# rland93/rrtplanner

Measured on NVIDIA B200. Metric: RRT* plans/sec (512x512 grid, n=5000), higher is better.
Workload: dtype f64

## Files before the change

profiles/region_profile.py:

```python
import csv, re, subprocess, sys, tempfile, os
sass_csv, so, cubin_name, func_pat = sys.argv[1:5]
tmp = tempfile.mkdtemp()
subprocess.check_call(["cuobjdump", "-xelf", "all", os.path.abspath(so)], cwd=tmp, stdout=subprocess.DEVNULL)
dis = subprocess.run(["nvdisasm", "-g", "-c", os.path.join(tmp, cubin_name)], capture_output=True, text=True).stdout
line_of = {}; cur=None; infunc=False
for ln in dis.splitlines():
    m = re.match(r"\s*\.section\s+\.text\.(\S+?),", ln)
    if m: infunc = func_pat in m.group(1); continue
    if not infunc: continue
    m = re.search(r'//## File "([^"]+)", line (\d+)(?: inlined at "([^"]+)", line (\d+))?', ln)
    if m:
        f, l = os.path.basename(m.group(1)), int(m.group(2))
        if m.group(3): of, ol = os.path.basename(m.group(3)), int(m.group(4))
        else: of, ol = None, None
        cur = (f, l, of, ol); continue
    m = re.match(r"\s*/\*([0-9a-f]{4,})\*/\s+(.*?);", ln)
    if m: line_of[int(m.group(1), 16)] = cur
rows = list(csv.reader(open(sass_csv))); hdr = rows[1]
ci, cs = hdr.index("Instructions Executed"), hdr.index("# Samples")
base = int(rows[2][0], 16)
regions = [("setup+prologue", 0, 178), ("owner:pickup", 179, 191), ("owner:scan", 192, 239), ("owner:nearest/dup/walk", 240, 287), ("owner:costing+cands", 288, 378), ("owner:record", 379, 392), ("commit", 393, 528), ("round end", 529, 543), ("goal+out", 544, 700)]
agg = {r[0]: [0, 0] for r in regions}; agg["other"] = [0, 0]; tot=[0,0]
unk = {}
for r in rows[2:]:
    try: off = int(r[0], 16) - base; n, s = int(r[ci]), int(r[cs])
    except Exception: continue
    k = line_of.get(off)
    line = None
    if k:
        if k[0] == "plan_grid.cuh": line = k[1]
        elif k[2] == "plan_grid.cuh": line = k[3]
    name = "other"
    if line is not None:
        for nm, a, b in regions:
            if a <= line <= b: name = nm
    else:
        unk[k] = unk.get(k, 0) + n
    agg[name][0] += n; agg[name][1] += s; tot[0]+=n; tot[1]+=s
for nm, (n, s) in agg.items(): print(f"{nm:28s} instr {n/1e6:8.1f}M {100*n/tot[0]:5.1f}%   samples {s:7d} {100*s/tot[1]:5.1f}%")
for k, n in sorted(unk.items(), key=lambda kv: -kv[1])[:12]: print("   other:", k, f"{n/1e6:.1f}M")
```

rrtplanner_b200/csrc/plan.cu:

```cuda
#include <cstdlib>

#include "plan_common.cuh"

namespace rrtk {

int scan_launch_standard(const PlanParams &, int, int, int, int, size_t, cudaStream_t);
int scan_launch_star(const PlanParams &, int, int, int, int, size_t, cudaStream_t);
int scan_launch_informed(const PlanParams &, int, int, int, int, size_t, cudaStream_t);
int scan_occupancy_standard(int, int, int, size_t);
int scan_occupancy_star(int, int, int, size_t);
int scan_occupancy_informed(int, int, int, size_t);
int grid_launch(int, int, const PlanParams &, int, size_t, cudaStream_t);
int grid_occupancy(int, int, bool, size_t);
int wide_plan_launch(int, const uint32_t *, int, int, const rrtk_plan_desc *, int, int, double, double, const int16_t *,
                     const double *, int16_t *, double *, int32_t *, int64_t *, double *, int, int, int, cudaStream_t);
int wide_plan_footprint(int, int, int, int, int, int, int, int *, int *);

struct ScanShape {
    int T, K, hit_words, tail_bytes, sbits, steps_max, list_cap, blocks_per_sm, two_per_sm;
    size_t smem;
};

static int env_int(const char *name, int dflt)
{
    const char *s = getenv(name);
    return (s && *s) ? atoi(s) : dflt;
}

#ifndef RRTK_MINB128
#define RRTK_MINB128 7
#endif
static int scan_min_blocks(int T) { return T <= 64 ? 12 : T <= 128 ? RRTK_MINB128 : T <= 160 ? 5 : T <= 256 ? 3 : 1; }

struct GridShape {
    int xb, yb, bshift, bshy, nbx, nby, rad, list_cap, blocks_per_sm, K, kb, ent_words, off_list, off_bstart;
    uint32_t near_ok2;
    size_t smem;
};

static int bits_for(int v) { int b = 0; while ((1 << b) <= v) ++b; return b; }

static bool grid_shape(int kind, int W, int H, int n, double r_rewire, int threads, int optin, int sm_smem, GridShape *out)
{
    const char *impl = getenv("RRTK_PLAN_IMPL");
    if (impl && (impl[0] == 'w' || impl[0] == 's')) return false;
#ifdef RRTK_GRID_OPT_IN
    if (!(impl && impl[0] == 'g')) return false;
#endif
    if (kind != RRTK_STANDARD && kind != RRTK_STAR) return false;
    if (threads != 0 && threads != 128) return false;
    if (env_int("RRTK_PLAN_T", 0) != 0) return false;
    if (n < 256 && !(impl && impl[0] == 'g')) return false;
    GridShape g;
    g.K = env_int("RRTK_GRID_K", 16);
    if (g.K != 8 && g.K != 16) return false;
    g.xb = bits_for(W - 1); g.yb = bits_for(H - 1);
    const int ib = 32 - g.xb - g.yb;
    if (ib < 1 || ib > 31 || (long long)n >= (1ll << ib) - 1) return false;
    g.bshift = env_int("RRTK_GRID_BSX", 5); g.bshy = env_int("RRTK_GRID_BSY", 2);
    for (;;) {
        g.nbx = (W + (1 << g.bshift) - 1) >> g.bshift; g.nby = (H + (1 << g.bshy) - 1) >> g.bshy;
        if (g.nbx * g.nby <= 2048 && g.nbx * g.nby + 1 <= n) break;
        if (g.bshift >= 15) return false;
        if (g.bshy < g.bshift) ++g.bshy; else ++g.bshift;
    }
    const double r = kind == RRTK_STAR ? (r_rewire > 0.0 ? r_rewire : 0.0) : 0.0;
    double rad = ceil(r);
    if (rad < (double)(1 << g.bshift)) rad = (double)(1 << g.bshift);
    if (rad > 32768.0) rad = 32768.0;
    g.rad = (int)rad;
    g.near_ok2 = (uint32_t)(rad * rad);
    int cap = env_int("RRTK_PLAN_CAP", 256);
    const int need = (n + 1 + 31) & ~31;
    g.list_cap = kind == RRTK_STANDARD ? 0 : (cap < need ? cap : need);
    g.ent_words = (n + 1 + 31) & ~31;
    g.off_list = 4 * g.ent_words;
    g.off_bstart = g.off_list + 4 * 4 * g.list_cap;
    g.smem = (size_t)g.off_bstart + (((size_t)2 * (g.nbx * g.nby + 1) + 15) & ~(size_t)15);
    g.kb = bits_for(n);
    {
        const long long d2max = (long long)(W - 1) * (W - 1) + (long long)(H - 1) * (H - 1);
        if (g.kb >= 32 || d2max >= (1ll << (32 - g.kb)) - 1 || env_int("RRTK_GRID_KEY32", 1) == 0) g.kb = 0;
    }
    if (g.smem > (size_t)optin - 4096) return false;
    int b = grid_occupancy(kind, g.K, g.kb > 0, g.smem);
    if (b <= 0) {
        b = (int)((size_t)sm_smem / (g.smem + 3072));
        if (b > 7) b = 7;
    }
    g.blocks_per_sm = b < 1 ? 1 : b;
    *out = g;
    return true;
}

static bool scan_shape(int kind, int W, int H, int n, int threads, int optin, int sm_smem, ScanShape *out)
{
    const char *impl = getenv("RRTK_PLAN_IMPL");
    if (impl && impl[0] == 'w') return false;
    if (n + 1 > 65535) return false;
    ScanShape s;
    s.K = env_int("RRTK_PLAN_K", 8);
    if (s.K != 4 && s.K != 8 && s.K != 16) return false;
    int T = threads > 0 ? threads : env_int("RRTK_PLAN_T", 0);
    if (T <= 0) T = n < 2048 ? 64 : n < 5120 ? 128 : n < 32768 ? 256 : 512;
    if (T != 64 && T != 128 && T != 160 && T != 256 && T != 512) return false;
    const int rows = (n + 1 + T - 1) / T;
    s.T = T;
    s.hit_words = (rows + 31) / 32;
    if (s.hit_words > 4) return false;
    s.sbits = s.hit_words == 1 ? 5 : s.hit_words == 2 ? 6 : 7;
    const long long side = W > H ? W : H;
    if (((2 * side * side) << s.sbits) > (1ll << 29)) return false;
    s.steps_max = (rows + 3) / 4;
    int cap = env_int("RRTK_PLAN_CAP", kind == RRTK_INFORMED ? 448 : 256);
    const int need = (n + 1 + 31) & ~31;
    s.list_cap = kind == RRTK_STANDARD ? 0 : (cap < need ? cap : need);
    s.smem = (size_t)4 * 4 * T * s.steps_max;
    const int tail_rows = rows - 32 * (s.hit_words - 1);
    s.tail_bytes = tail_rows <= 8 ? 1 : tail_rows <= 16 ? 2 : 4;
    if (kind != RRTK_STANDARD)
        s.smem += (size_t)4 * (s.hit_words - 1) * s.K * T + (((size_t)s.tail_bytes * s.K * T + 3) & ~(size_t)3) + (size_t)2 * (T / 32) * s.list_cap;
    s.smem = (s.smem + 15) & ~(size_t)15;
    if (s.smem > (size_t)optin - 2048) return false;
    s.two_per_sm = (T == 256 && (size_t)sm_smem / (s.smem + 2048) <= 2) ? 1 : 0;
    int b = kind == RRTK_STANDARD ? scan_occupancy_standard(T, s.K, s.two_per_sm, s.smem)
            : kind == RRTK_STAR   ? scan_occupancy_star(T, s.K, s.two_per_sm, s.smem)
                                  : scan_occupancy_informed(T, s.K, s.two_per_sm, s.smem);
    if (b <= 0) {
        const int by_smem = (int)((size_t)sm_smem / (s.smem + 1024 + 1024));
        const int by_threads = 2048 / T;
        b = by_smem < by_threads ? by_smem : by_threads;
        const int mb = s.two_per_sm ? 2 : scan_min_blocks(T);
        const int by_regs = 65536 / (T * (65536 / (T * mb) / 8 * 8));
        if (b > by_regs) b = by_regs;
    }
    s.blocks_per_sm = b < 1 ? 1 : (b > 32 ? 32 : b);
    *out = s;
    return true;
}

const char *plan_kernel_name(int kind, int W, int H, int n, int threads, int optin, int sm_smem)
{
    GridShape g;
    if (grid_shape(kind, W, H, n, 0.0, threads, optin, sm_smem, &g)) return "grid";
    ScanShape s;
    return scan_shape(kind, W, H, n, threads, optin, sm_smem, &s) ? "scan" : "wide";
}

int plan_footprint(int kind, int W, int H, int n, int threads, int optin, int sm_smem, int *smem_bytes, int *blocks_per_sm)
{
    GridShape g;
    if (grid_shape(kind, W, H, n, 0.0, threads, optin, sm_smem, &g)) {
        if (smem_bytes) *smem_bytes = (int)g.smem;
        if (blocks_per_sm) *blocks_per_sm = g.blocks_per_sm;
        return RRTK_OK;
    }
    ScanShape s;
    if (!scan_shape(kind, W, H, n, threads, optin, sm_smem, &s))
        return wide_plan_footprint(kind, W, H, n, threads == 160 || threads == 512 ? 0 : threads, optin, sm_smem, smem_bytes, blocks_per_sm);
    if (smem_bytes) *smem_bytes = (int)s.smem;
    if (blocks_per_sm) *blocks_per_sm = s.blocks_per_sm;
    return RRTK_OK;
}

int plan_launch(int kind, const uint32_t *d_bits, int W, int H, const rrtk_plan_desc *d_plans, int nplans, int n,
                double r_rewire, double r_goal, const int16_t *d_samples, const double *d_balls, int16_t *d_pts,
                double *d_cost, int32_t *d_parent, int64_t *d_stats, double *d_ell_c, int threads, int optin,
                int sm_smem, cudaStream_t st)
{
    if (kind != RRTK_STANDARD && kind != RRTK_STAR && kind != RRTK_INFORMED) {
        set_error("unknown planner kind %d", kind);
        return RRTK_ERR_INVALID;
    }
    GridShape g;
    const bool use_grid = grid_shape(kind, W, H, n, r_rewire, threads, optin, sm_smem, &g);
    ScanShape s;
    if (!use_grid && !scan_shape(kind, W, H, n, threads, optin, sm_smem, &s))
        return wide_plan_launch(kind, d_bits, W, H, d_plans, nplans, n, r_rewire, r_goal, d_samples, d_balls, d_pts, d_cost,
                                d_parent, d_stats, d_ell_c, threads == 160 || threads == 512 ? 0 : threads, optin, sm_smem, st);
    PlanParams P;
    P.bits = d_bits;
    P.words_per_grid = grid_words(W, H);
    P.W = W; P.H = H; P.TY = tiles_y(H);
    P.plans = d_plans;
    P.n = n;
    const double lim = ceil(r_rewire * r_rewire);
    P.r2_excl = (kind == RRTK_STANDARD) ? 0u : (lim >= 1073741824.0 ? 1073741824u : (lim <= 0.0 ? 0u : (uint32_t)lim));
    P.r_goal = r_goal;
    P.samples = reinterpret_cast<const short2 *>(d_samples);
    P.balls = reinterpret_cast<const double2 *>(d_balls);
    P.pts = reinterpret_cast<short2 *>(d_pts);
    P.cost = d_cost;
    P.parent = d_parent;
    P.stats = reinterpret_cast<long long *>(d_stats);
    P.ell_c = d_ell_c;
    if (use_grid) {
        P.sbits = 0; P.hit_words = 0; P.tail_bytes = 0; P.steps_max = 0;
        P.list_cap = g.list_cap;
        P.g_xb = g.xb; P.g_yb = g.yb; P.g_bshift = g.bshift; P.g_bshy = g.bshy; P.g_nbx = g.nbx; P.g_nby = g.nby; P.g_rad = g.rad; P.g_near_ok2 = g.near_ok2;
        P.g_ent_words = g.ent_words; P.g_off_list = g.off_list; P.g_off_bstart = g.off_bstart; P.g_kb = g.kb;
        return grid_launch(kind, g.K, P, nplans, g.smem, st);
    }
    P.g_xb = P.g_yb = P.g_bshift = P.g_bshy = P.g_nbx = P.g_nby = P.g_rad = 0; P.g_near_ok2 = 0;
    P.g_ent_words = P.g_off_list = P.g_off_bstart = P.g_kb = 0;
    P.sbits = s.sbits;
    P.list_cap = s.list_cap;
    P.hit_words = s.hit_words;
    P.tail_bytes = s.tail_bytes;
    P.steps_max = s.steps_max;
    switch (kind) {
        case RRTK_STANDARD: return scan_launch_standard(P, nplans, s.T, s.K, s.two_per_sm, s.smem, st);
        case RRTK_STAR: return scan_launch_star(P, nplans, s.T, s.K, s.two_per_sm, s.smem, st);
        default: return scan_launch_informed(P, nplans, s.T, s.K, s.two_per_sm, s.smem, st);
    }
}

__global__ void paths_kernel(const int *parent, const long long *stats, int nplans, int n, int cap, int *path, int *len)
{
    const int p = blockIdx.x * blockDim.x + threadIdx.x;
    if (p >= nplans) return;
    const int *par = parent + (size_t)p * (n + 1);
    int *out = path + (size_t)p * cap;
    int v = (int)stats[(size_t)p * RRTK_STAT_COUNT + RRTK_STAT_VGOAL];
    int depth = 0;
    for (int u = v; u > 0 && depth <= n; u = par[u]) ++depth;
    const int L = depth + 1;
    len[p] = L;
    if (L > cap) return;
    int u = v;
    for (int k = L - 1; k >= 0; --k) { out[k] = u; u = u > 0 ? par[u] : 0; }
}

__global__ void paths_xy_kernel(const int *parent, const short2 *pts, const double *cost, const long long *stats, int nplans, int n,
                                int cap, int *path, short2 *xy, int *len, double *pcost)
{
    const int p = blockIdx.x * blockDim.x + threadIdx.x;
    if (p >= nplans) return;
    const size_t row = (size_t)p * (n + 1);
    const int *par = parent + row;
    int v = (int)stats[(size_t)p * RRTK_STAT_COUNT + RRTK_STAT_VGOAL];
    int depth = 0;
    for (int u = v; u > 0 && depth <= n; u = par[u]) ++depth;
    const int L = depth + 1;
    len[p] = L;
    pcost[p] = cost[row + v];
    if (L > cap) return;
    int u = v;
    for (int k = L - 1; k >= 0; --k) {
        path[(size_t)p * cap + k] = u;
        xy[(size_t)p * cap + k] = pts[row + u];
        u = u > 0 ? par[u] : 0;
    }
    for (int k = L; k < cap; ++k) { path[(size_t)p * cap + k] = -1; xy[(size_t)p * cap + k] = make_short2(-32768, -32768); }
}

int paths_xy_launch(const int32_t *d_parent, const int16_t *d_pts, const double *d_cost, const int64_t *d_stats, int nplans, int n, int cap,
                    int32_t *d_path, int16_t *d_xy, int32_t *d_len, double *d_pcost, cudaStream_t st)
{
    paths_xy_kernel<<<(nplans + 127) / 128, 128, 0, st>>>(d_parent, reinterpret_cast<const short2 *>(d_pts), d_cost,
                                                         reinterpret_cast<const long long *>(d_stats), nplans, n, cap, d_path,
                                                         reinterpret_cast<short2 *>(d_xy), d_len, d_pcost);
    RRTK_CUDA(cudaGetLastError());
    return RRTK_OK;
}

__global__ void path_heads_kernel(const int *path, const uint8_t *head, int nplans, int n, int cap, uint8_t *out)
{
    const size_t i = blockIdx.x * (size_t)blockDim.x + threadIdx.x;
    if (i >= (size_t)nplans * cap) return;
    const int v = path[i];
    out[i] = v < 0 ? (uint8_t)255 : head[(i / cap) * (size_t)(n + 1) + v];
}

int path_heads_launch(const int32_t *d_path, const uint8_t *d_head, int nplans, int n, int cap, uint8_t *d_out, cudaStream_t st)
{
    const size_t total = (size_t)nplans * cap;
    if (total == 0) return RRTK_OK;
    path_heads_kernel<<<(unsigned)((total + 255) / 256), 256, 0, st>>>(d_path, d_head, nplans, n, cap, d_out);
    RRTK_CUDA(cudaGetLastError());
    return RRTK_OK;
}

int paths_launch(const int32_t *d_parent, const int64_t *d_stats, int nplans, int n, int cap, int32_t *d_path,
                 int32_t *d_len, cudaStream_t st)
{
    paths_kernel<<<(nplans + 127) / 128, 128, 0, st>>>(d_parent, reinterpret_cast<const long long *>(d_stats), nplans, n,
                                                      cap, d_path, d_len);
    RRTK_CUDA(cudaGetLastError());
    return RRTK_OK;
}

}
```

rrtplanner_b200/csrc/plan_common.cuh:

```cuda
#pragma once
#include <math_constants.h>

#include "common.cuh"

namespace rrtk {

struct PlanParams {
    const uint32_t *bits;
    size_t words_per_grid;
    int W, H, TY;
    const rrtk_plan_desc *plans;
    int n;
    uint32_t r2_excl;
    double r_goal;
    const short2 *samples;
    const double2 *balls;
    short2 *pts;
    double *cost;
    int *parent;
    long long *stats;
    double *ell_c;
    int sbits;
    int list_cap;
    int hit_words;
    int tail_bytes;
    int steps_max;
    int g_xb, g_yb;
    int g_bshift, g_bshy;
    int g_nbx, g_nby;
    int g_rad;
    uint32_t g_near_ok2;
    int g_ent_words, g_off_list, g_off_bstart;
    int g_kb;
};

struct SampleRec {
    uint32_t pnew;
    uint32_t bd;
    int vnear;
    int flags;
    int bv;
    int ring;
    double c0;
    double bc;
    double ell;
};

struct RoundSummary {
    int j, consumed, flags;
    int vsol;
    int kwant, pad;
    double csol;
    long long first_sol;
};

__device__ __forceinline__ unsigned warp_min_u32(unsigned v) { return __reduce_min_sync(RRTK_FULL, v); }

__device__ __forceinline__ void ellipse_sample(int W, int H, const double *rot, int sx, int sy, int gx, int gy,
                                               double c, double2 ball, int &ox, int &oy)
{
    const double cx = __ddiv_rn((double)(sx + gx), 2.0), cy = __ddiv_rn((double)(sy + gy), 2.0);
    const double r1 = __ddiv_rn(c, 2.0);
    const long long ddx = sx - gx, ddy = sy - gy;
    const double d2 = (double)(ddx * ddx + ddy * ddy);
    const double r2 = __ddiv_rn(__dsqrt_rn(fabs(__dsub_rn(__dmul_rn(c, c), d2))), 2.0);
    const double m00 = __dmul_rn(rot[0], r1), m01 = __dmul_rn(rot[1], r2);
    const double m10 = __dmul_rn(rot[2], r1), m11 = __dmul_rn(rot[3], r2);
    const double x = __dadd_rn(__dadd_rn(__dmul_rn(m00, ball.x), __dmul_rn(m01, ball.y)), cx);
    const double y = __dadd_rn(__dadd_rn(__dmul_rn(m10, ball.x), __dmul_rn(m11, ball.y)), cy);
    double lx = (x < (double)(W - 1)) ? x : (double)(W - 1);
    double ly = (y < (double)(H - 1)) ? y : (double)(H - 1);
    lx = (lx > 0.0) ? lx : 0.0;
    ly = (ly > 0.0) ? ly : 0.0;
    ox = (int)lx;
    oy = (int)ly;
}


}
```

rrtplanner_b200/csrc/plan_grid.cuh:

```cuda
#pragma once
#include "plan_common.cuh"

namespace rrtk {

constexpr uint32_t kSlotEmpty = 0xffffffffu;
constexpr int kFirst = 256;

#ifndef RRTK_GRID_MINB
#define RRTK_GRID_MINB 7
#endif

template <int KIND, int K, int T, bool KEY32>
__global__ void __launch_bounds__(T, RRTK_GRID_MINB) plan_grid_kernel(PlanParams P)
{
    constexpr int NW = T / 32;
    static_assert(T % 32 == 0 && K <= 16 && K >= 1, "block shape");
    static_assert(KIND == RRTK_STANDARD || KIND == RRTK_STAR, "the samples of an informed plan are not known in advance");
    extern __shared__ __align__(16) uint32_t smem[];
    __shared__ SampleRec s_rec[K];
    __shared__ RoundSummary s_sum;
    __shared__ short2 s_q[K];
    __shared__ int s_sig[K];
    __shared__ int s_next;
    __shared__ int s_rootslot;
    __shared__ unsigned long long s_goalc;
    __shared__ int s_goalv;
    __shared__ unsigned long long s_checks, s_cells;
    __shared__ unsigned long long s_cnt[4];
    __shared__ uint32_t s_first[kFirst];

    const int tid = threadIdx.x;
    const int lane = tid & 31, warp = tid >> 5;
    const int plan = blockIdx.x;
    const int n = P.n;
    const int cap = P.list_cap;
    const int nslots = n + 1;
    const int xb = P.g_xb, xyb = P.g_xb + P.g_yb;
    const uint32_t xmask = (1u << P.g_xb) - 1u, ymask = (1u << P.g_yb) - 1u;
    const int bsx = P.g_bshift, bsy = P.g_bshy, NBY = P.g_nby, NB = P.g_nbx * P.g_nby, rr = P.g_rad;
    const uint32_t near_ok2 = P.g_near_ok2;

    uint32_t *s_ent = smem;
    const int ent_words = P.g_ent_words;
    uint32_t *s_list = reinterpret_cast<uint32_t *>(reinterpret_cast<unsigned char *>(smem) + P.g_off_list);
    uint16_t *s_bstart = reinterpret_cast<uint16_t *>(reinterpret_cast<unsigned char *>(smem) + P.g_off_bstart);
    const int kb = P.g_kb;
    short2 *opts = P.pts + (size_t)plan * (n + 1);

    const rrtk_plan_desc *dsc = P.plans + plan;
    const uint32_t *gbits = P.bits + (size_t)dsc->world * P.words_per_grid;
    const int sx = dsc->start_x, sy = dsc->start_y, gx = dsc->goal_x, gy = dsc->goal_y;

    double *cost = P.cost + (size_t)plan * (n + 1);
    int *parent = P.parent + (size_t)plan * (n + 1);
    const short2 *samples = P.samples + (size_t)plan * n;
    const uint32_t r2x = P.r2_excl;

    auto bucket_of = [&](int x, int y) { return (x >> bsx) * NBY + (y >> bsy); };
    auto make_entry = [&](int x, int y, int id) { return ((uint32_t)id << xyb) | ((uint32_t)y << xb) | (uint32_t)x; };
    auto ent_xy = [&](uint32_t e) { return pack_xy((int)(e & xmask), (int)((e >> xb) & ymask)); };
    auto ent_id = [&](uint32_t e) { return (int)(e >> xyb); };

    {
        uint32_t *cnt = s_ent;
        for (int b = tid; b <= NB; b += T) cnt[b] = 0u;
        __syncthreads();
        for (int i = tid; i <= n; i += T) {
            const short2 q = i < n ? samples[i] : make_short2((short)sx, (short)sy);
            atomicAdd(&cnt[bucket_of(q.x, q.y)], 1u);
        }
        __syncthreads();
        if (warp == 0) {
            uint32_t run = 0;
            for (int base = 0; base <= NB; base += 32) {
                const int b = base + lane;
                const uint32_t c = b < NB ? cnt[b] : 0u;
                uint32_t incl = c;
#pragma unroll
                for (int o = 1; o < 32; o <<= 1) {
                    const uint32_t t = __shfl_up_sync(RRTK_FULL, incl, o);
                    if (lane >= o) incl += t;
                }
                if (b <= NB) { s_bstart[b] = (uint16_t)(run + incl - c); cnt[b] = run + incl - c; }
                run += __shfl_sync(RRTK_FULL, incl, 31);
            }
        }
        __syncthreads();
        for (int i = tid; i <= n; i += T) {
            const short2 q = i < n ? samples[i] : make_short2((short)sx, (short)sy);
            const int slot = (int)atomicAdd(&cnt[bucket_of(q.x, q.y)], 1u);
            if (i < n) parent[i + 1] = slot;
            else s_rootslot = slot;
        }
        __syncthreads();
        for (int i = tid; i < ent_words; i += T) s_ent[i] = kSlotEmpty;
        for (int i = tid; i < kFirst; i += T) s_first[i] = kSlotEmpty;
        __syncthreads();
    }
    if (tid < K) {
        const int i0 = min(tid, n - 1);
        s_q[tid] = samples[i0];
        s_sig[tid] = parent[i0 + 1];
    }
    if (tid == 0) {
        const uint32_t e0 = make_entry(sx, sy, 0);
        s_ent[s_rootslot] = e0; s_first[0] = e0;
        opts[0] = make_short2((short)sx, (short)sy);
        s_next = NW;
        s_checks = s_cells = 0ull; cost[0] = 0.0; parent[0] = -1;
    }
    if (tid < 4) s_cnt[tid] = 0ull;
    __syncthreads();

    GlobalGrid gg{gbits};
    const int TY = P.TY;
#define WALK(ax_, ay_, bx_, by_) warp_first_hit(gg, TY, ax_, ay_, bx_, by_, lane)

    int j = 1, it0 = 0, kwant = 1;
    int cw = 0;
    unsigned my_checks = 0, my_cells = 0;
    const unsigned ltmask = (1u << lane) - 1u;
#ifdef RRTK_PHASE_CLOCKS
    long long clk_scan = 0, clk_owner = 0, clk_commit = 0, clk_ownwork = 0, rounds = 0;
#define GPHASE_T(var) const long long var = clock64()
#define GPHASE_ADD(acc, a, b) acc += (b) - (a)
#else
#define GPHASE_T(var)
#define GPHASE_ADD(acc, a, b)
#endif

    while (it0 < n) {
        GPHASE_T(t_0);
        if (j == n) break;
        const int kact = min(min(K, n - it0), kwant);
        short2 ahead = make_short2(0, 0);
        int ahead_sig = 0;
        if (warp == cw && lane < 2 * K) {
            const int ia = min(it0 + lane, n - 1);
            ahead = samples[ia];
            ahead_sig = parent[ia + 1];
        }

        for (int k = warp; k < K;) {
            if (k >= kact) {
                if (lane == 0) s_rec[k].flags = 0;
                int nk = 0;
                if (lane == 0) nk = atomicAdd(&s_next, 1);
                k = __shfl_sync(RRTK_FULL, nk, 0);
                continue;
            }
            const short2 smp = s_q[k];
            const int x = smp.x, y = smp.y;
            uint32_t *list = s_list + warp * cap;
            GPHASE_T(t_s0);
            uint32_t bd = 0xffffffffu, bv = 0xffffffffu, be = 0u;
            int total = 0;
            constexpr int kVis = 1;
            auto visit = [&](const uint32_t *src, int base, int end, bool members) {
                const int idx = base + lane;
                const uint32_t e = idx < end ? src[idx] : kSlotEmpty;
                const int dx = (int)(e & xmask) - x, dy = (int)((e >> xb) & ymask) - y;
                const bool valid = e != kSlotEmpty;
                const uint32_t d2r = (uint32_t)(dx * dx + dy * dy);
                const uint32_t id = e >> xyb;
                bool mem;
                if (KEY32) {
                    const uint32_t key = valid ? (d2r << kb) + id : 0xffffffffu;
                    bd = min(bd, key);
                    mem = valid && d2r < r2x;
                } else {
                    const uint32_t d2 = valid ? d2r : 0xffffffffu;
                    if (d2 < bd || (d2 == bd && id < bv)) { bd = d2; bv = id; be = e; }
                    mem = d2 < r2x;
                }
                if (KIND != RRTK_STANDARD && members) {
                    const unsigned mm = __ballot_sync(RRTK_FULL, mem);
                    const int at = total + __popc(mm & ltmask);
                    if (mem && at < cap) list[at] = e;
                    total += __popc(mm);
                }
            };
            auto nearest_d2 = [&]() { const uint32_t m = __reduce_min_sync(RRTK_FULL, bd); return KEY32 ? (m >> kb) : m; };
            __syncwarp();
            if (j <= kFirst) {
                for (int base = 0; base < j; base += 32 * kVis) visit(s_first, base, j, true);
            } else {
                const int bx0 = max(x - rr, 0) >> bsx, bx1 = min(x + rr, P.W - 1) >> bsx;
                const int by0 = max(y - rr, 0) >> bsy, by1 = min(y + rr, P.H - 1) >> bsy;
                for (int bxx = bx0; bxx <= bx1; ++bxx) {
                    const int s0 = s_bstart[bxx * NBY + by0], s1 = s_bstart[bxx * NBY + by1 + 1];
                    for (int base = s0; base < s1; base += 32 * kVis) visit(s_ent, base, s1, true);
                }
                if (nearest_d2() > near_ok2) {
                    for (int base = 0; base < nslots; base += 32 * kVis) visit(s_ent, base, nslots, false);
                }
            }
            __syncwarp();
            GPHASE_T(t_s1);
            GPHASE_ADD(clk_scan, t_s0, t_s1);
            int vnear;
            uint32_t pnear;
            if (KEY32) {
                const uint32_t mk = __reduce_min_sync(RRTK_FULL, bd);
                bd = mk >> kb;
                vnear = (int)(mk & ((1u << kb) - 1u));
                const short2 pn = opts[vnear];
                pnear = pack_xy(pn.x, pn.y);
            } else {
                const uint32_t md = __reduce_min_sync(RRTK_FULL, bd);
                const uint32_t mv = __reduce_min_sync(RRTK_FULL, bd == md ? bv : 0xffffffffu);
                const uint32_t near_e = __shfl_sync(RRTK_FULL, be, __ffs(__ballot_sync(RRTK_FULL, bd == md && bv == mv)) - 1);
                bd = md;
                vnear = (int)mv;
                pnear = ent_xy(near_e);
            }
            bool dup = bd == 0 && vnear >= 1;
            if (bd == 0 && vnear == 0) {
                bool f = false;
                if (j <= kFirst) {
                    for (int v = 1 + lane; v < j; v += 32) f |= ent_xy(s_first[v]) == pack_xy(x, y);
                } else {
                    const int b = bucket_of(x, y);
                    for (int s = s_bstart[b] + lane; s < s_bstart[b + 1]; s += 32) {
                        const uint32_t e = s_ent[s];
                        f |= e != kSlotEmpty && ent_id(e) >= 1 && ent_xy(e) == pack_xy(x, y);
                    }
                }
                dup = __any_sync(RRTK_FULL, f);
            }
            int flags = 1 | (dup ? 2 : 0);
            double c0 = 0.0, wc = CUDART_INF;
            int wv = 0x7fffffff, ring = 0;
            if (!dup) {
                const double cnear = cost[vnear];
                const int hit = WALK(px(pnear), py(pnear), x, y);
                my_checks += 1; my_cells += cells_tested(hit);
                if (hit < 0) {
                    flags |= 4;
                    c0 = reach_cost(cnear, bd);
                    if (KIND != RRTK_STANDARD) {
                        ring = total;
                        if (total <= cap) {
                            for (int base = 0; base < total; base += 96) {
                                int cv[3];
                                uint32_t cp[3];
                                unsigned long long ck[3];
                                double ccv[3];
                                const int left = total - base;
#pragma unroll
                                for (int u = 0; u < 3; ++u) {
                                    ck[u] = ~0ull; cv[u] = 0; cp[u] = 0u; ccv[u] = CUDART_INF;
                                    if (32 * u < left) {
                                        const int idx = base + 32 * u + lane;
                                        const bool has = idx < total;
                                        const uint32_t e = has ? list[idx] : 0u;
                                        cv[u] = ent_id(e);
                                        cp[u] = ent_xy(e);
                                        if (has) ccv[u] = cost[cv[u]];
                                    }
                                }
#pragma unroll
                                for (int u = 0; u < 3; ++u) {
                                    if (32 * u < left) {
                                        const double cn = reach_cost(ccv[u], dist2(cp[u], x, y));
                                        const bool live = cn < c0 && (cn < wc || (cn == wc && cv[u] < wv));
                                        if (live) ck[u] = (unsigned long long)__double_as_longlong(cn);
                                    }
                                }
                                for (;;) {
                                    unsigned long long bk = ck[0];
                                    int bu = 0, bvx = cv[0];
                                    if (ck[1] < bk || (ck[1] == bk && cv[1] < bvx)) { bk = ck[1]; bu = 1; bvx = cv[1]; }
                                    if (ck[2] < bk || (ck[2] == bk && cv[2] < bvx)) { bk = ck[2]; bu = 2; bvx = cv[2]; }
                                    const uint32_t hi = (uint32_t)(bk >> 32);
                                    const uint32_t mhi = warp_min_u32(hi);
                                    if (mhi == 0xffffffffu) break;
                                    const uint32_t lo = (hi == mhi) ? (uint32_t)bk : 0xffffffffu;
                                    const uint32_t mlo = warp_min_u32(lo);
                                    const uint32_t vv = (hi == mhi && lo == mlo) ? (uint32_t)bvx : 0xffffffffu;
                                    const uint32_t mvv = warp_min_u32(vv);
                                    const int src = __ffs(__ballot_sync(RRTK_FULL, vv == mvv)) - 1;
                                    const uint32_t bpx = bu == 0 ? cp[0] : bu == 1 ? cp[1] : cp[2];
                                    const uint32_t pp = __shfl_sync(RRTK_FULL, bpx, src);
                                    const int h = WALK(px(pp), py(pp), x, y);
                                    my_checks += 1; my_cells += cells_tested(h);
                                    if (h < 0) { wc = __hiloint2double((int)mhi, (int)mlo); wv = (int)mvv; break; }
                                    if (lane == src) {
                                        if (bu == 0) ck[0] = ~0ull; else if (bu == 1) ck[1] = ~0ull; else ck[2] = ~0ull;
                                    }
                                }
                            }
                        } else {
                            auto consider = [&](bool has, int v, uint32_t p, double cn) {
                                bool live = has && cn < c0;
                                for (;;) {
                                    const bool cand = live && (cn < wc || (cn == wc && v < wv));
                                    if (!__any_sync(RRTK_FULL, cand)) break;
                                    const uint32_t hi = cand ? (uint32_t)__double2hiint(cn) : 0xffffffffu;
                                    const uint32_t mhi = warp_min_u32(hi);
                                    const uint32_t lo = (cand && hi == mhi) ? (uint32_t)__double2loint(cn) : 0xffffffffu;
                                    const uint32_t mlo = warp_min_u32(lo);
                                    const uint32_t vv = (cand && hi == mhi && lo == mlo) ? (uint32_t)v : 0xffffffffu;
                                    const uint32_t mvv = warp_min_u32(vv);
                                    const int src = __ffs(__ballot_sync(RRTK_FULL, vv == mvv && mvv != 0xffffffffu)) - 1;
                                    const uint32_t pp = __shfl_sync(RRTK_FULL, p, src);
                                    const int h = WALK(px(pp), py(pp), x, y);
                                    my_checks += 1; my_cells += cells_tested(h);
                                    if (h < 0) { wc = __hiloint2double((int)mhi, (int)mlo); wv = (int)mvv; }
                                    else if (lane == src) live = false;
                                }
                            };
                            for (int base = 0; base < nslots; base += 32) {
                                const uint32_t e = base + lane < nslots ? s_ent[base + lane] : kSlotEmpty;
                                const bool valid = e != kSlotEmpty;
                                const uint32_t p = ent_xy(e);
                                const uint32_t dd = dist2(p, x, y);
                                const int v = ent_id(e);
                                const bool has = valid && dd < r2x;
                                double cn = CUDART_INF;
                                if (has) cn = reach_cost(cost[v], dd);
                                consider(has, v, p, cn);
                            }
                        }
                    }
                }
            }
            if (lane == 0) {
                SampleRec r;
                r.pnew = pack_xy(x, y); r.bd = bd; r.vnear = vnear; r.flags = flags; r.bv = wv; r.ring = ring;
                r.c0 = c0; r.bc = wc; r.ell = 0.0;
                s_rec[k] = r;
            }
            {
                int nk = 0;
                if (lane == 0) nk = atomicAdd(&s_next, 1);
                k = __shfl_sync(RRTK_FULL, nk, 0);
            }
        }
        GPHASE_T(t_1b);
        __syncthreads();
        GPHASE_T(t_2);

        if (warp == cw) {
            uint32_t newp = 0;
            double newc = 0.0;
            int nnew = 0, consumed = 0, jc = j;
            bool finished = false;
            bool fast = false;
            auto insert = [&](int v, uint32_t pnew, int slot) {
                const uint32_t e = make_entry(px(pnew), py(pnew), v);
                s_ent[slot] = e;
                if (v < kFirst) s_first[v] = e;
                if (KEY32) opts[v] = make_short2((short)px(pnew), (short)py(pnew));
            };
            if (j + kact <= n) {
                const SampleRec r = s_rec[min(lane, K - 1)];
                const int myslot = s_sig[min(lane, K - 1)];
                const bool in = lane < kact;
                bool a = in && !(r.flags & 2) && (r.flags & 4);
                double bc = r.bc;
                int bv = r.bv;
                const int x = px(r.pnew), y = py(r.pnew);
                int extra = 0, stop = kact, nacc = 0;
                unsigned addm = __ballot_sync(RRTK_FULL, a);
                for (int kk = 0; kk < stop; ++kk) {
                    if (!((addm >> kk) & 1u)) continue;
                    const uint32_t pk = __shfl_sync(RRTK_FULL, r.pnew, kk);
                    const uint32_t du = dist2(pk, x, y);
                    const bool later = in && lane > kk && lane < stop;
                    if (!__any_sync(RRTK_FULL, later && (du < r.bd || (a && (du == 0 || du < r2x))))) { ++nacc; continue; }
                    const double myc = (bv != 0x7fffffff) ? bc : r.c0;
                    const double ck = __shfl_sync(RRTK_FULL, myc, kk);
                    const unsigned cutm = __ballot_sync(RRTK_FULL, later && du != 0 && du < r.bd);
                    if (cutm) stop = min(stop, __ffs(cutm) - 1);
                    const bool still = later && lane < stop;
                    if (still && du == 0 && a) a = false;
                    addm = __ballot_sync(RRTK_FULL, a);
                    const bool inr = KIND != RRTK_STANDARD && still && a && du < r2x;
                    if (__any_sync(RRTK_FULL, inr)) {
                        double cn = CUDART_INF;
                        if (inr) { ++extra; cn = reach_cost(ck, du); }
                        unsigned wm = __ballot_sync(RRTK_FULL, inr && cn < r.c0 && cn < bc);
                        while (wm) {
                            const int dst = __ffs(wm) - 1;
                            wm &= wm - 1;
                            const uint32_t pq = __shfl_sync(RRTK_FULL, r.pnew, dst);
                            const int h = WALK(px(pk), py(pk), px(pq), py(pq));
                            my_checks += 1; my_cells += cells_tested(h);
                            if (h < 0 && lane == dst) { bc = cn; bv = j + nacc; }
                        }
                    }
                    ++nacc;
                }
                const bool cons = lane < stop;
                const bool acc = a && cons;
                const unsigned accm = __ballot_sync(RRTK_FULL, acc);
                const int myj = j + __popc(accm & ltmask);
                if (acc) {
                    const bool hasbv = bv != 0x7fffffff;
                    insert(myj, r.pnew, myslot);
                    cost[myj] = hasbv ? bc : r.c0; parent[myj] = hasbv ? bv : r.vnear;
                }
                consumed = stop;
                jc = j + __popc(accm);
                const int np_ = __reduce_add_sync(RRTK_FULL, cons ? myj : 0), rm_ = __reduce_add_sync(RRTK_FULL, acc ? r.ring + extra : 0);
                if (lane == 0) { s_cnt[1] += (unsigned long long)np_; s_cnt[2] += (unsigned long long)rm_; s_cnt[3] += (unsigned long long)__popc(accm); }
                fast = true;
            }
            for (int k = 0; k < kact && !fast; ++k) {
                const SampleRec r = s_rec[k];
                if (jc == n) { finished = true; break; }
                const int x = px(r.pnew), y = py(r.pnew);
                bool reject = (r.flags & 2) || jc == n || !(r.flags & 4);
                double bc = r.bc;
                int bv = r.bv;
                const bool mine = lane < nnew;
                const uint32_t du = mine ? dist2(newp, x, y) : 0xffffffffu;
                if (__any_sync(RRTK_FULL, mine && du != 0 && du < r.bd)) break;
                if (__any_sync(RRTK_FULL, mine && du == 0)) reject = true;
                int ringm = r.ring;
                if (KIND != RRTK_STANDARD && !reject) {
                    const bool inr = mine && du < r2x;
                    const unsigned inm = __ballot_sync(RRTK_FULL, inr);
                    ringm += __popc(inm);
                    if (inm) {
                        double cn = CUDART_INF;
                        if (inr) cn = reach_cost(newc, du);
                        bool live = inr && cn < r.c0 && cn < bc;
                        for (;;) {
                            if (!__any_sync(RRTK_FULL, live)) break;
                            const uint32_t hi = live ? (uint32_t)__double2hiint(cn) : 0xffffffffu;
                            const uint32_t mhi = warp_min_u32(hi);
                            const uint32_t lo = (live && hi == mhi) ? (uint32_t)__double2loint(cn) : 0xffffffffu;
                            const uint32_t mlo = warp_min_u32(lo);
                            const int src = __ffs(__ballot_sync(RRTK_FULL, live && hi == mhi && lo == mlo)) - 1;
                            const uint32_t pp = __shfl_sync(RRTK_FULL, newp, src);
                            const int h = WALK(px(pp), py(pp), x, y);
                            my_checks += 1; my_cells += cells_tested(h);
                            if (h < 0) { bc = __hiloint2double((int)mhi, (int)mlo); bv = j + src; break; }
                            if (lane == src) live = false;
                        }
                    }
                }
                ++consumed;
                if (lane == 0) s_cnt[1] += (unsigned long long)jc;
                if (reject) continue;
                if (lane == 0) { s_cnt[2] += (unsigned long long)ringm; s_cnt[3] += 1ull; }
                const int vbest = (bv != 0x7fffffff) ? bv : r.vnear;
                const double cbest = (bv != 0x7fffffff) ? bc : r.c0;
                if (lane == 0) { insert(jc, r.pnew, s_sig[k]); cost[jc] = cbest; parent[jc] = vbest; }
                if (lane == nnew) { newp = r.pnew; newc = cbest; }
                ++nnew;
                ++jc;
            }
            if (it0 + consumed >= n) finished = true;
            __syncwarp();
            const int kwant_next = consumed < kact ? max(min(K, 1 + (jc >> 3)), max(1, kact >> 1)) : min(K, 2 * kact);
            if (lane == 0) s_next = NW;
            {
                const int src = min(consumed + lane, 31);
                const int ax_ = __shfl_sync(RRTK_FULL, (int)ahead.x, src), ay_ = __shfl_sync(RRTK_FULL, (int)ahead.y, src);
                const int sg_ = __shfl_sync(RRTK_FULL, ahead_sig, src);
                if (lane < K) { s_q[lane] = make_short2((short)ax_, (short)ay_); s_sig[lane] = sg_; }
            }
            if (lane == 0) {
                RoundSummary s;
                s.j = jc; s.consumed = consumed; s.flags = finished ? 2 : 0;
                s.vsol = 0; s.csol = 0.0; s.first_sol = -1;
                s.kwant = kwant_next; s.pad = 0;
                s_sum = s;
            }
        }
        __syncthreads();
        GPHASE_T(t_3);
        GPHASE_ADD(clk_owner, t_0, t_2); GPHASE_ADD(clk_commit, t_2, t_3); GPHASE_ADD(clk_ownwork, t_0, t_1b);
#ifdef RRTK_PHASE_CLOCKS
        ++rounds;
#endif
        {
            const RoundSummary s = s_sum;
            cw = (cw + 1 == NW) ? 0 : cw + 1;
            j = s.j;
            it0 += s.consumed;
            kwant = s.kwant;
            if (s.flags & 2) break;
        }
    }

    if (tid == 0) { s_goalc = 0x7ff0000000000000ull; s_goalv = 0x7fffffff; }
    __syncthreads();
    for (int base = warp * 32; base < nslots; base += NW * 32) {
        const uint32_t e = base + lane < nslots ? s_ent[base + lane] : kSlotEmpty;
        const bool valid = e != kSlotEmpty;
        const uint32_t p = ent_xy(e);
        double cg = CUDART_INF;
        if (valid) cg = reach_cost(cost[ent_id(e)], dist2(p, gx, gy));
        unsigned m = __ballot_sync(RRTK_FULL, valid && cg < __longlong_as_double(*(volatile unsigned long long *)&s_goalc));
        while (m) {
            const int l = __ffs(m) - 1;
            m &= m - 1;
            const double cv = __shfl_sync(RRTK_FULL, cg, l);
            const uint32_t pp = __shfl_sync(RRTK_FULL, p, l);
            if (cv < __longlong_as_double(*(volatile unsigned long long *)&s_goalc)) {
                const int h = WALK(px(pp), py(pp), gx, gy);
                my_checks += 1; my_cells += cells_tested(h);
                if (h < 0 && lane == 0) atomicMin(&s_goalc, (unsigned long long)__double_as_longlong(cv));
            }
        }
    }
    __syncthreads();
    const unsigned long long cstar_bits = s_goalc;
    const bool reachable = cstar_bits != 0x7ff0000000000000ull;
    if (reachable) {
        for (int base = warp * 32; base < nslots; base += NW * 32) {
            const uint32_t e = base + lane < nslots ? s_ent[base + lane] : kSlotEmpty;
            const bool valid = e != kSlotEmpty;
            const uint32_t p = ent_xy(e);
            const int v = ent_id(e);
            double cg = CUDART_INF;
            if (valid) cg = reach_cost(cost[v], dist2(p, gx, gy));
            unsigned m = __ballot_sync(RRTK_FULL, valid && (unsigned long long)__double_as_longlong(cg) == cstar_bits);
            while (m) {
                const int l = __ffs(m) - 1;
                m &= m - 1;
                const uint32_t pp = __shfl_sync(RRTK_FULL, p, l);
                const int vv = __shfl_sync(RRTK_FULL, v, l);
                const int h = WALK(px(pp), py(pp), gx, gy);
                my_checks += 1; my_cells += cells_tested(h);
                if (h < 0 && lane == 0) atomicMin(&s_goalv, vv);
            }
        }
    }
    if (lane == 0) {
        atomicAdd(&s_checks, (unsigned long long)my_checks);
        atomicAdd(&s_cells, (unsigned long long)my_cells);
    }
    __syncthreads();

    const int vparent = s_goalv;
    const bool found = reachable && vparent != 0x7fffffff;
    const int top = found ? j + 1 : j;
    for (int v = j + tid; v <= n; v += T) {
        opts[v] = (v == j && found) ? make_short2((short)gx, (short)gy) : make_short2(-32768, -32768);
        if (v >= top) { cost[v] = CUDART_INF; parent[v] = -1; }
    }
    if (!KEY32)
        for (int s = tid; s < nslots; s += T) {
            const uint32_t e = s_ent[s];
            if (e != kSlotEmpty) opts[ent_id(e)] = make_short2((short)(e & xmask), (short)((e >> xb) & ymask));
        }
    __syncthreads();
    if (tid == 0) {
        if (found) { cost[j] = __longlong_as_double((long long)cstar_bits); parent[j] = vparent; }
        long long *st = P.stats + (size_t)plan * RRTK_STAT_COUNT;
        st[RRTK_STAT_J] = j;
        st[RRTK_STAT_VGOAL] = found ? j : 0;
        st[RRTK_STAT_FOUND] = found ? 1 : 0;
        st[RRTK_STAT_CHECKS] = (long long)s_checks;
        st[RRTK_STAT_CELLS] = (long long)s_cells;
        st[RRTK_STAT_FIRST_SOL_ITER] = -1;
        st[RRTK_STAT_ELL_ITERS] = 0;
        st[RRTK_STAT_NN_PAIRS] = (long long)s_cnt[1];
        st[RRTK_STAT_RING_MEMBERS] = (long long)s_cnt[2];
        st[RRTK_STAT_ACCEPTED] = (long long)s_cnt[3];
        st[RRTK_STAT_RESERVED0] = 0;
        st[RRTK_STAT_RESERVED1] = 0;
#ifdef RRTK_PHASE_CLOCKS
        st[RRTK_STAT_RESERVED0] = clk_scan;
        st[RRTK_STAT_RESERVED1] = clk_owner;
        st[RRTK_STAT_ELL_ITERS] = clk_commit;
        st[RRTK_STAT_FIRST_SOL_ITER] = clk_ownwork;
        st[RRTK_STAT_RING_MEMBERS] = rounds;
#endif
    }
#undef WALK
}

}
```

Before: 113,100.

## Periodically rebuild compact bucketed slot layout over accepted nodes plus upcoming samples

New measurement: 121,400, median of 6. +7.4%, better.

```diff
diff --git a/profiles/region_profile.py b/profiles/region_profile.py
--- a/profiles/region_profile.py
+++ b/profiles/region_profile.py
@@ -19,7 +19,7 @@
 rows = list(csv.reader(open(sass_csv))); hdr = rows[1]
 ci, cs = hdr.index("Instructions Executed"), hdr.index("# Samples")
 base = int(rows[2][0], 16)
-regions = [("setup+prologue", 0, 178), ("owner:pickup", 179, 191), ("owner:scan", 192, 239), ("owner:nearest/dup/walk", 240, 287), ("owner:costing+cands", 288, 378), ("owner:record", 379, 392), ("commit", 393, 528), ("round end", 529, 543), ("goal+out", 544, 700)]
+regions = [("re-layout", 51, 114), ("setup+prologue", 115, 207), ("owner:pickup", 208, 236), ("owner:scan", 237, 289), ("owner:nearest/dup/walk", 290, 332), ("owner:costing+cands", 333, 426), ("owner:record", 427, 439), ("commit", 440, 577), ("round end", 578, 592), ("goal+out", 593, 700)]
 agg = {r[0]: [0, 0] for r in regions}; agg["other"] = [0, 0]; tot=[0,0]
 unk = {}
 for r in rows[2:]:
diff --git a/rrtplanner_b200/csrc/plan.cu b/rrtplanner_b200/csrc/plan.cu
--- a/rrtplanner_b200/csrc/plan.cu
+++ b/rrtplanner_b200/csrc/plan.cu
@@ -33,7 +33,7 @@
 static int scan_min_blocks(int T) { return T <= 64 ? 12 : T <= 128 ? RRTK_MINB128 : T <= 160 ? 5 : T <= 256 ? 3 : 1; }
 
 struct GridShape {
-    int xb, yb, bshift, bshy, nbx, nby, rad, list_cap, blocks_per_sm, K, kb, ent_words, off_list, off_bstart;
+    int xb, yb, bshift, bshy, nbx, nby, rad, list_cap, blocks_per_sm, K, kb, ent_words, off_list, off_bstart, stretch;
     uint32_t near_ok2;
     size_t smem;
 };
@@ -54,6 +54,8 @@
     GridShape g;
     g.K = env_int("RRTK_GRID_K", 16);
     if (g.K != 8 && g.K != 16) return false;
+    const int stretch = env_int("RRTK_GRID_RELAYOUT", 768);
+    g.stretch = (stretch <= 0 || stretch >= n) ? n : stretch;
     g.xb = bits_for(W - 1); g.yb = bits_for(H - 1);
     const int ib = 32 - g.xb - g.yb;
     if (ib < 1 || ib > 31 || (long long)n >= (1ll << ib) - 1) return false;
@@ -198,11 +200,12 @@
         P.sbits = 0; P.hit_words = 0; P.tail_bytes = 0; P.steps_max = 0;
         P.list_cap = g.list_cap;
         P.g_xb = g.xb; P.g_yb = g.yb; P.g_bshift = g.bshift; P.g_bshy = g.bshy; P.g_nbx = g.nbx; P.g_nby = g.nby; P.g_rad = g.rad; P.g_near_ok2 = g.near_ok2;
-        P.g_ent_words = g.ent_words; P.g_off_list = g.off_list; P.g_off_bstart = g.off_bstart; P.g_kb = g.kb;
+        P.g_off_list = g.off_list; P.g_off_bstart = g.off_bstart; P.g_kb = g.kb;
+        P.g_stretch = g.stretch;
         return grid_launch(kind, g.K, P, nplans, g.smem, st);
     }
     P.g_xb = P.g_yb = P.g_bshift = P.g_bshy = P.g_nbx = P.g_nby = P.g_rad = 0; P.g_near_ok2 = 0;
-    P.g_ent_words = P.g_off_list = P.g_off_bstart = P.g_kb = 0;
+    P.g_off_list = P.g_off_bstart = P.g_kb = P.g_stretch = 0;
     P.sbits = s.sbits;
     P.list_cap = s.list_cap;
     P.hit_words = s.hit_words;
diff --git a/rrtplanner_b200/csrc/plan_common.cuh b/rrtplanner_b200/csrc/plan_common.cuh
--- a/rrtplanner_b200/csrc/plan_common.cuh
+++ b/rrtplanner_b200/csrc/plan_common.cuh
@@ -30,8 +30,9 @@
     int g_nbx, g_nby;
     int g_rad;
     uint32_t g_near_ok2;
-    int g_ent_words, g_off_list, g_off_bstart;
+    int g_off_list, g_off_bstart;
     int g_kb;
+    int g_stretch;
 };
 
 struct SampleRec {
diff --git a/rrtplanner_b200/csrc/plan_grid.cuh b/rrtplanner_b200/csrc/plan_grid.cuh
--- a/rrtplanner_b200/csrc/plan_grid.cuh
+++ b/rrtplanner_b200/csrc/plan_grid.cuh
@@ -9,6 +9,60 @@
 #ifndef RRTK_GRID_MINB
 #define RRTK_GRID_MINB 7
 #endif
+
+template <int K, int T>
+__device__ __noinline__ void grid_relayout(int it0, int j, int end, int NB, int NBY, int bsx, int bsy, int xb, int xyb,
+                                           const short2 *opts, const short2 *samples, int *parent, uint32_t *s_ent,
+                                           uint16_t *s_bstart, short2 *s_q, int *s_sig, uint32_t *s_wsum, int *s_nslots)
+{
+    const int tid = threadIdx.x, lane = tid & 31, warp = tid >> 5;
+    const int L = j + (end - it0);
+    uint32_t *cnt = reinterpret_cast<uint32_t *>(s_bstart);
+    const int nw = (NB + 2) >> 1;
+    auto bucket_of = [&](short2 q) { return (q.x >> bsx) * NBY + (q.y >> bsy); };
+    auto point = [&](int i) { return i < j ? opts[i] : samples[it0 + i - j]; };
+    for (int w = tid; w < nw; w += T) cnt[w] = 0u;
+    for (int i = tid; i < L; i += T) s_ent[i] = kSlotEmpty;
+    __syncthreads();
+    for (int i = tid; i < L; i += T) {
+        const int b = bucket_of(point(i));
+        atomicAdd(&cnt[b >> 1], 1u << ((b & 1) << 4));
+    }
+    __syncthreads();
+    const int per = (nw + T - 1) / T, w0 = min(tid * per, nw), w1 = min(w0 + per, nw);
+    uint32_t sum = 0;
+    for (int w = w0; w < w1; ++w) { const uint32_t c = cnt[w]; sum += (c & 0xffffu) + (c >> 16); }
+    uint32_t incl = sum;
+#pragma unroll
+    for (int o = 1; o < 32; o <<= 1) {
+        const uint32_t t = __shfl_up_sync(RRTK_FULL, incl, o);
+        if (lane >= o) incl += t;
+    }
+    if (lane == 31) s_wsum[warp] = incl;
+    __syncthreads();
+    uint32_t run = incl - sum;
+    for (int w = 0; w < warp; ++w) run += s_wsum[w];
+    for (int w = w0; w < w1; ++w) {
+        const uint32_t c = cnt[w], lo = run + (c & 0xffffu);
+        run = lo + (c >> 16);
+        cnt[w] = lo | (run << 16);
+    }
+    __syncthreads();
+    for (int i = tid; i < L; i += T) {
+        const short2 q = point(i);
+        const int b = bucket_of(q), sh = (b & 1) << 4;
+        const int slot = (int)((atomicAdd(&cnt[b >> 1], 0u - (1u << sh)) >> sh) & 0xffffu) - 1;
+        if (i < j) {
+            s_ent[slot] = ((uint32_t)i << xyb) | ((uint32_t)q.y << xb) | (uint32_t)q.x;
+        } else {
+            const int k = i - j;
+            parent[it0 + k + 1] = slot;
+            if (k < K) { s_q[k] = q; s_sig[k] = slot; }
+        }
+    }
+    if (tid == 0) *s_nslots = L;
+    __syncthreads();
+}
 
 template <int KIND, int K, int T, bool KEY32>
 __global__ void __launch_bounds__(T, RRTK_GRID_MINB) plan_grid_kernel(PlanParams P)
@@ -22,7 +76,8 @@
     __shared__ short2 s_q[K];
     __shared__ int s_sig[K];
     __shared__ int s_next;
-    __shared__ int s_rootslot;
+    __shared__ int s_nslots;
+    __shared__ uint32_t s_wsum[NW];
     __shared__ unsigned long long s_goalc;
     __shared__ int s_goalv;
     __shared__ unsigned long long s_checks, s_cells;
@@ -34,14 +89,13 @@
     const int plan = blockIdx.x;
     const int n = P.n;
     const int cap = P.list_cap;
-    const int nslots = n + 1;
+    const int stretch = P.g_stretch;
     const int xb = P.g_xb, xyb = P.g_xb + P.g_yb;
     const uint32_t xmask = (1u << P.g_xb) - 1u, ymask = (1u << P.g_yb) - 1u;
     const int bsx = P.g_bshift, bsy = P.g_bshy, NBY = P.g_nby, NB = P.g_nbx * P.g_nby, rr = P.g_rad;
     const uint32_t near_ok2 = P.g_near_ok2;
 
     uint32_t *s_ent = smem;
-    const int ent_words = P.g_ent_words;
     uint32_t *s_list = reinterpret_cast<uint32_t *>(reinterpret_cast<unsigned char *>(smem) + P.g_off_list);
     uint16_t *s_bstart = reinterpret_cast<uint16_t *>(reinterpret_cast<unsigned char *>(smem) + P.g_off_bstart);
     const int kb = P.g_kb;
@@ -61,56 +115,21 @@
     auto ent_xy = [&](uint32_t e) { return pack_xy((int)(e & xmask), (int)((e >> xb) & ymask)); };
     auto ent_id = [&](uint32_t e) { return (int)(e >> xyb); };
 
-    {
-        uint32_t *cnt = s_ent;
-        for (int b = tid; b <= NB; b += T) cnt[b] = 0u;
-        __syncthreads();
-        for (int i = tid; i <= n; i += T) {
-            const short2 q = i < n ? samples[i] : make_short2((short)sx, (short)sy);
-            atomicAdd(&cnt[bucket_of(q.x, q.y)], 1u);
-        }
-        __syncthreads();
-        if (warp == 0) {
-            uint32_t run = 0;
-            for (int base = 0; base <= NB; base += 32) {
-                const int b = base + lane;
-                const uint32_t c = b < NB ? cnt[b] : 0u;
-                uint32_t incl = c;
-#pragma unroll
-                for (int o = 1; o < 32; o <<= 1) {
-                    const uint32_t t = __shfl_up_sync(RRTK_FULL, incl, o);
-                    if (lane >= o) incl += t;
-                }
-                if (b <= NB) { s_bstart[b] = (uint16_t)(run + incl - c); cnt[b] = run + incl - c; }
-                run += __shfl_sync(RRTK_FULL, incl, 31);
-            }
-        }
-        __syncthreads();
-        for (int i = tid; i <= n; i += T) {
-            const short2 q = i < n ? samples[i] : make_short2((short)sx, (short)sy);
-            const int slot = (int)atomicAdd(&cnt[bucket_of(q.x, q.y)], 1u);
-            if (i < n) parent[i + 1] = slot;
-            else s_rootslot = slot;
-        }
-        __syncthreads();
-        for (int i = tid; i < ent_words; i += T) s_ent[i] = kSlotEmpty;
-        for (int i = tid; i < kFirst; i += T) s_first[i] = kSlotEmpty;
-        __syncthreads();
-    }
-    if (tid < K) {
-        const int i0 = min(tid, n - 1);
-        s_q[tid] = samples[i0];
-        s_sig[tid] = parent[i0 + 1];
-    }
+    for (int i = tid; i < kFirst; i += T) s_first[i] = kSlotEmpty;
     if (tid == 0) {
-        const uint32_t e0 = make_entry(sx, sy, 0);
-        s_ent[s_rootslot] = e0; s_first[0] = e0;
         opts[0] = make_short2((short)sx, (short)sy);
         s_next = NW;
         s_checks = s_cells = 0ull; cost[0] = 0.0; parent[0] = -1;
     }
     if (tid < 4) s_cnt[tid] = 0ull;
     __syncthreads();
+    if (tid == 0) s_first[0] = make_entry(sx, sy, 0);
+    int limit = min(n, stretch);
+#define RELAYOUT() grid_relayout<K, T>(it0, j, limit, NB, NBY, bsx, bsy, xb, xyb, opts, samples, parent, s_ent, s_bstart, s_q, s_sig, s_wsum, &s_nslots)
+    {
+        const int it0 = 0, j = 1;
+        RELAYOUT();
+    }
 
     GlobalGrid gg{gbits};
     const int TY = P.TY;
@@ -132,7 +151,11 @@
     while (it0 < n) {
         GPHASE_T(t_0);
         if (j == n) break;
-        const int kact = min(min(K, n - it0), kwant);
+        if (limit < n && it0 + 2 * K > limit) {
+            limit = min(n, it0 + stretch);
+            RELAYOUT();
+        }
+        const int kact = min(min(K, limit - it0), kwant);
         short2 ahead = make_short2(0, 0);
         int ahead_sig = 0;
         if (warp == cw && lane < 2 * K) {
@@ -192,6 +215,7 @@
                     for (int base = s0; base < s1; base += 32 * kVis) visit(s_ent, base, s1, true);
                 }
                 if (nearest_d2() > near_ok2) {
+                    const int nslots = s_nslots;
                     for (int base = 0; base < nslots; base += 32 * kVis) visit(s_ent, base, nslots, false);
                 }
             }
@@ -310,6 +334,7 @@
                                     else if (lane == src) live = false;
                                 }
                             };
+                            const int nslots = s_nslots;
                             for (int base = 0; base < nslots; base += 32) {
                                 const uint32_t e = base + lane < nslots ? s_ent[base + lane] : kSlotEmpty;
                                 const bool valid = e != kSlotEmpty;
@@ -351,7 +376,7 @@
                 const uint32_t e = make_entry(px(pnew), py(pnew), v);
                 s_ent[slot] = e;
                 if (v < kFirst) s_first[v] = e;
-                if (KEY32) opts[v] = make_short2((short)px(pnew), (short)py(pnew));
+                opts[v] = make_short2((short)px(pnew), (short)py(pnew));
             };
             if (j + kact <= n) {
                 const SampleRec r = s_rec[min(lane, K - 1)];
@@ -489,6 +514,7 @@
 
     if (tid == 0) { s_goalc = 0x7ff0000000000000ull; s_goalv = 0x7fffffff; }
     __syncthreads();
+    const int nslots = s_nslots;
     for (int base = warp * 32; base < nslots; base += NW * 32) {
         const uint32_t e = base + lane < nslots ? s_ent[base + lane] : kSlotEmpty;
         const bool valid = e != kSlotEmpty;
@@ -544,11 +570,6 @@
         opts[v] = (v == j && found) ? make_short2((short)gx, (short)gy) : make_short2(-32768, -32768);
         if (v >= top) { cost[v] = CUDART_INF; parent[v] = -1; }
     }
-    if (!KEY32)
-        for (int s = tid; s < nslots; s += T) {
-            const uint32_t e = s_ent[s];
-            if (e != kSlotEmpty) opts[ent_id(e)] = make_short2((short)(e & xmask), (short)((e >> xb) & ymask));
-        }
     __syncthreads();
     if (tid == 0) {
         if (found) { cost[j] = __longlong_as_double((long long)cstar_bits); parent[j] = vparent; }
@@ -574,6 +595,7 @@
 #endif
     }
 #undef WALK
+#undef RELAYOUT
 }
 
 }
```
